# Quantus-Network/qp-zk-circuits

Measured on AMD Instinct MI355X. Metric: Wormhole proofs/sec, higher is better.
Workload: dtype u64

## Files before the change

include/qpgpu.h:

```cpp
#ifndef QPGPU_H
#define QPGPU_H
#include <stddef.h>
#include <stdint.h>

#ifdef __cplusplus
extern "C" {
#endif

typedef struct qpgpu_ctx qpgpu_ctx;
typedef struct qpgpu_circuit qpgpu_circuit;

enum {
    QPGPU_OK = 0,
    QPGPU_EINVAL = -1,
    QPGPU_EDEVICE = -2,
    QPGPU_ENOMEM = -3,
    QPGPU_EUNSAT = -4,
    QPGPU_EBUFSIZE = -5
};

int qpgpu_ctx_create(int device, qpgpu_ctx **out);
void qpgpu_ctx_destroy(qpgpu_ctx *ctx);
const char *qpgpu_last_error(const qpgpu_ctx *ctx);
int qpgpu_ctx_set_stream(qpgpu_ctx *ctx, void *hip_stream);
// ... 40 lines not shown
                           unsigned log_leaves, unsigned cap_height, uint64_t *d_digests, uint64_t *h_cap_out);
int qpgpu_merkle_build_rows_dev(qpgpu_ctx *ctx, const uint64_t *d_rows, uint32_t width, unsigned log_leaves,
                                unsigned cap_height, uint64_t *d_digests, uint64_t *h_cap_out);

int qpgpu_circuit_load(qpgpu_ctx *ctx, const uint64_t *pack_words, size_t n_words, qpgpu_circuit **out);
int qpgpu_circuit_load_batch(qpgpu_ctx *ctx, const uint64_t *pack_words, size_t n_words, unsigned max_batch, qpgpu_circuit **out);
unsigned qpgpu_circuit_max_batch(const qpgpu_circuit *c);
size_t qpgpu_circuit_num_public_inputs(const qpgpu_circuit *c);
void qpgpu_circuit_free(qpgpu_circuit *c);
int qpgpu_circuit_scrub(qpgpu_circuit *c);
int qpgpu_circuit_constants_sigmas_cap(const qpgpu_circuit *c, uint64_t *out, size_t out_words);
int qpgpu_circuit_set_blinding_seed(qpgpu_circuit *c, uint64_t seed);
int qpgpu_circuit_set_witness_check(qpgpu_circuit *c, int on);
int qpgpu_circuit_set_quotient_fused(qpgpu_circuit *c, int on);
int qpgpu_circuit_quotient_info(const qpgpu_circuit *c, int *fused_enabled, int *fused_selected);
size_t qpgpu_proof_size(const qpgpu_circuit *c);
int qpgpu_prove(qpgpu_circuit *c, const uint64_t *wires, const uint64_t *public_inputs, uint8_t *out, size_t out_cap, size_t *out_len);
int qpgpu_prove_dev(qpgpu_circuit *c, const uint64_t *d_wires, const uint64_t *public_inputs, uint8_t *out, size_t out_cap, size_t *out_len);
int qpgpu_prove_batch_dev(qpgpu_circuit *c, const uint64_t *const *d_wires, uint32_t batch, const uint64_t *const *public_inputs,
                          uint8_t *const *outs, size_t out_cap, size_t *out_lens);

int qpgpu_witness_info(qpgpu_circuit *c, uint64_t *num_generators, uint64_t *num_levels, uint64_t *num_free_cells);
int qpgpu_witness_free_mask(qpgpu_circuit *c, uint8_t *mask, size_t mask_len);
int qpgpu_generate_witness_dev(qpgpu_circuit *c, uint64_t *d_wires, const uint64_t *public_inputs);
int qpgpu_generate_witness(qpgpu_circuit *c, uint64_t *wires, const uint64_t *public_inputs);
int qpgpu_circuit_gate_rows(const qpgpu_circuit *c, unsigned gate_type, uint32_t *rows_out, size_t cap, size_t *count);
int qpgpu_generate_witness_batch_dev(qpgpu_circuit *c, uint64_t *d_wires, uint32_t batch, const uint64_t *public_inputs);
int qpgpu_generate_witness_partial_dev(qpgpu_circuit *c, const uint64_t *cells, const uint64_t *values, size_t count,
                                       const uint64_t *public_inputs, uint64_t *d_wires);
int qpgpu_generate_witness_partial_batch_dev(qpgpu_circuit *c, const uint64_t *cells, size_t count, const uint64_t *values,
// ... 143 lines not shown
```

integration/qpgpu_backend.rs:

```rust

use anyhow::{anyhow, bail, Result};
use core::ffi::{c_char, c_void};
use plonky2::field::extension::Extendable;
use plonky2::field::polynomial::PolynomialCoeffs;
use plonky2::field::types::PrimeField64;
use plonky2::hash::hash_types::RichField;
use plonky2::iop::target::Target;
use plonky2::iop::witness::{PartialWitness, PartitionWitness};
use plonky2::plonk::circuit_data::{CircuitData, CommonCircuitData, ProverOnlyCircuitData};
use plonky2::plonk::config::GenericConfig;
use plonky2::plonk::proof::ProofWithPublicInputs;

#[repr(C)] pub struct QpgpuCtx { _p: [u8; 0] }
#[repr(C)] pub struct QpgpuCircuit { _p: [u8; 0] }
#[repr(C)] pub struct QpgpuOracle { _p: [u8; 0] }
#[repr(C)] pub struct QpgpuStagePlan { _p: [u8; 0] }
#[repr(C)] pub struct QpgpuFriSession { _p: [u8; 0] }
#[repr(C)] pub struct QpgpuChallenger { pub sponge_state: [u64; 12], pub input_buffer: [u64; 8], pub output_buffer: [u64; 8], pub input_len: u32, pub output_len: u32 }
#[repr(C)] pub struct QpgpuFriRange { pub oracle: u32, pub first: u32, pub count: u32 }
#[repr(C)] pub struct QpgpuFriBatch { pub point: [u64; 2], pub num_ranges: u32, pub ranges: [QpgpuFriRange; 8] }
#[repr(C)] pub struct QpgpuFriParams { pub rate_bits: u32, pub cap_height: u32, pub proof_of_work_bits: u32, pub num_query_rounds: u32,
                                       pub num_reduction_rounds: u32, pub reduction_arity_bits: [u32; 16] }
pub const QPGPU_STAGE_ERR_CAP: usize = 256;

// ... 3 lines not shown
#[link(name = "qpgpu")]
extern "C" {
    pub fn qpgpu_ctx_create(device: i32, out: *mut *mut QpgpuCtx) -> i32;
    pub fn qpgpu_ctx_destroy(ctx: *mut QpgpuCtx);
    pub fn qpgpu_last_error(ctx: *const QpgpuCtx) -> *const c_char;
    pub fn qpgpu_ctx_pci_bus_id(ctx: *const QpgpuCtx, out: *mut c_char, out_len: usize) -> i32;
    pub fn qpgpu_ctx_set_hasher(ctx: *mut QpgpuCtx, kind: i32, params: *const u64, n_words: usize) -> i32;
    pub fn qpgpu_malloc(ctx: *mut QpgpuCtx, bytes: usize, dptr: *mut *mut c_void) -> i32;
    pub fn qpgpu_free(ctx: *mut QpgpuCtx, dptr: *mut c_void) -> i32;
    pub fn qpgpu_free_scrubbed(ctx: *mut QpgpuCtx, dptr: *mut c_void, bytes: usize) -> i32;
    pub fn qpgpu_memcpy_h2d(ctx: *mut QpgpuCtx, dst: *mut c_void, src: *const c_void, bytes: usize) -> i32;
    pub fn qpgpu_circuit_load_batch(ctx: *mut QpgpuCtx, pack: *const u64, n_words: usize, max_batch: u32, out: *mut *mut QpgpuCircuit) -> i32;
    pub fn qpgpu_circuit_free(c: *mut QpgpuCircuit);
    pub fn qpgpu_circuit_scrub(c: *mut QpgpuCircuit) -> i32;
    pub fn qpgpu_circuit_set_witness_check(c: *mut QpgpuCircuit, on: i32) -> i32;
    pub fn qpgpu_proof_size(c: *const QpgpuCircuit) -> usize;
    pub fn qpgpu_prove(c: *mut QpgpuCircuit, wires: *const u64, public_inputs: *const u64, out: *mut u8, out_cap: usize, out_len: *mut usize) -> i32;
    pub fn qpgpu_generate_witness_partial_dev(c: *mut QpgpuCircuit, cells: *const u64, values: *const u64, count: usize,
                                              public_inputs: *const u64, d_wires: *mut u64) -> i32;
    pub fn qpgpu_prove_dev(c: *mut QpgpuCircuit, d_wires: *const u64, public_inputs: *const u64, out: *mut u8, out_cap: usize, out_len: *mut usize) -> i32;
    pub fn qpgpu_prove_batch_dev(c: *mut QpgpuCircuit, d_wires: *const *const u64, batch: u32, public_inputs: *const *const u64,
                                 outs: *const *mut u8, out_cap: usize, out_lens: *mut usize) -> i32;
    pub fn qpgpu_pack_validate(pack: *const u64, n_words: usize, err: *mut c_char) -> i32;
    pub fn qpgpu_stage_plan_create(ctx: *mut QpgpuCtx, words: *const u64, n_words: usize, cs_oracle: *const QpgpuOracle,
                                   out: *mut *mut QpgpuStagePlan, err: *mut c_char) -> i32;
    pub fn qpgpu_stage_plan_free(plan: *mut QpgpuStagePlan);
    pub fn qpgpu_stage_plan_info(plan: *const QpgpuStagePlan, degree_bits: *mut u32, num_challenges: *mut u32, num_partial_products: *mut u32,
                                 quotient_degree_factor: *mut u32, fused_selected: *mut i32) -> i32;
    pub fn qpgpu_stage_partial_products(plan: *mut QpgpuStagePlan, wires: *const u64, wires_on_device: i32, betas: *const u64,
                                        gammas: *const u64, d_out: *mut u64) -> i32;
// ... 537 lines not shown
```

qp-zk-circuits_amd/binding.py:

```python
import ctypes
import os

import numpy as np

P = 0xFFFFFFFF00000001
MULT_GEN = 14293326489335486720

NTT_FORWARD = 0
NTT_INVERSE = 1
NTT_OUT_BITREV = 2

_HERE = os.path.dirname(os.path.abspath(__file__))


def lib_path():
    return os.path.join(_HERE, "libqpgpu.so")


class QpGpuError(RuntimeError):
    def __init__(self, code, msg):
        super().__init__(f"qpgpu error {code}: {msg}")
        self.code = code


# ... 68 lines not shown
        "qpgpu_circuit_max_batch": (c.c_uint, [vp]),
        "qpgpu_circuit_scrub": (c.c_int, [vp]),
        "qpgpu_prove_batch_dev": (c.c_int, [vp, vp, c.c_uint32, vp, vp, c.c_size_t, vp]),
        "qpgpu_ctx_set_hasher": (c.c_int, [vp, c.c_int, u64p, c.c_size_t]),
        "qpgpu_ctx_get_hasher": (c.c_int, [vp]),
        "qpgpu_ctx_challenger_observe": (c.c_int, [vp, vp, u64p, c.c_size_t]),
        "qpgpu_ctx_challenger_get": (c.c_int, [vp, vp, c.POINTER(c.c_uint64)]),
        "qpgpu_pool_create_batched": (c.c_int, [c.c_int, u64p, c.c_size_t, c.c_uint, c.c_uint, c.POINTER(vp)]),
        "qpgpu_circuit_free": (None, [vp]),
        "qpgpu_circuit_constants_sigmas_cap": (c.c_int, [vp, u64p, c.c_size_t]),
        "qpgpu_proof_size": (c.c_size_t, [vp]),
        "qpgpu_circuit_set_blinding_seed": (c.c_int, [vp, c.c_uint64]),
        "qpgpu_circuit_set_witness_check": (c.c_int, [vp, c.c_int]),
        "qpgpu_circuit_set_quotient_fused": (c.c_int, [vp, c.c_int]),
        "qpgpu_circuit_quotient_info": (c.c_int, [vp, c.POINTER(c.c_int), c.POINTER(c.c_int)]),
        "qpgpu_circuit_gate_rows": (c.c_int, [vp, c.c_uint, vp, c.c_size_t, c.POINTER(c.c_size_t)]),
        "qpgpu_prove": (c.c_int, [vp, u64p, u64p, vp, c.c_size_t, c.POINTER(c.c_size_t)]),
        "qpgpu_prove_dev": (c.c_int, [vp, u64p, u64p, vp, c.c_size_t, c.POINTER(c.c_size_t)]),
        "qpgpu_poseidon_constants": (c.c_size_t, [u64p, u64p, c.c_size_t]),
        "qpgpu_pool_create": (c.c_int, [c.c_int, u64p, c.c_size_t, c.c_uint, c.POINTER(vp)]),
        "qpgpu_pool_destroy": (None, [vp]),
        "qpgpu_pool_proof_size": (c.c_size_t, [vp]),
        "qpgpu_pool_workers": (c.c_uint, [vp]),
        "qpgpu_pool_last_error": (c.c_char_p, [vp]),
        "qpgpu_pool_submit": (c.c_int, [vp, u64p, u64p, vp, c.c_size_t, c.POINTER(c.c_uint64)]),
        "qpgpu_pool_wait": (c.c_int, [vp, c.c_uint64, c.POINTER(c.c_size_t)]),
        "qpgpu_pool_set_witness_check": (c.c_int, [vp, c.c_int]),
        "qpgpu_pool_create_multi": (c.c_int, [vp, c.c_uint, u64p, c.c_size_t, c.c_uint, c.c_uint, c.c_uint, c.POINTER(vp)]),
        "qpgpu_pool_devices": (c.c_uint, [vp]),
        "qpgpu_pool_serialized": (c.c_int, [vp]),
# ... 357 lines not shown

    def proof_size(self):
        return self.gpu.lib.qpgpu_proof_size(self.h)

    def set_witness_check(self, on=True):
        self.gpu._check(self.gpu.lib.qpgpu_circuit_set_witness_check(self.h, 1 if on else 0))

    def set_quotient_fused(self, on=True):
        self.gpu._check(self.gpu.lib.qpgpu_circuit_set_quotient_fused(self.h, 1 if on else 0))

    def quotient_info(self):
        a, b = ctypes.c_int(), ctypes.c_int()
        self.gpu._check(self.gpu.lib.qpgpu_circuit_quotient_info(self.h, ctypes.byref(a), ctypes.byref(b)))
        return bool(a.value), bool(b.value)

    def set_blinding_seed(self, seed):
        self.gpu._check(self.gpu.lib.qpgpu_circuit_set_blinding_seed(self.h, seed))

    def constants_sigmas_cap(self, cap_height=4):
        out = np.empty((1 << cap_height, 4), dtype=np.uint64)
        self.gpu._check(self.gpu.lib.qpgpu_circuit_constants_sigmas_cap(self.h, out.ctypes.data, out.size))
        return out

    def witness_info(self):
        a, b, c3 = ctypes.c_uint64(), ctypes.c_uint64(), ctypes.c_uint64()
        self.gpu._check(self.gpu.lib.qpgpu_witness_info(self.h, ctypes.byref(a), ctypes.byref(b), ctypes.byref(c3)))
        return a.value, b.value, c3.value

    def gate_rows(self, gate_type):
        n = ctypes.c_size_t()
# ... 761 lines not shown
```

qp-zk-circuits_amd/csrc/prover.cpp:

```cpp
#include <hip/hip_runtime.h>
#include <algorithm>
#include <array>
#include <cstring>
#include <random>
#include <string>
#include <vector>
#include "circuit.hpp"
#include "ctx.hpp"
#include "gl64.hpp"
#include "merkle.hpp"
#include "poseidon.hpp"
#include "prover_host.hpp"
#include "circuit_state.hpp"
#include "prover_kernels.hpp"

using gl::e2;
using gl::u64;

namespace {

int alloc_batch(qpgpu_circuit *c, PolyOracle &b, uint32_t ncols, uint32_t nb, bool need_coeffs = true, uint32_t oracle_index = 0) {
    const CircuitPack &p = c->pack;
    const u64 n = p.n(), lde_n = n << p.rate_bits;
    const bool secret = oracle_index > 0;
// ... 158 lines not shown
}

int qpgpu_circuit_set_quotient_fused(qpgpu_circuit *c, int on) {
    if (!c) return QPGPU_EINVAL;
    c->tab.quotient_fused = on != 0;
    return QPGPU_OK;
}

int qpgpu_circuit_quotient_info(const qpgpu_circuit *c, int *fused_enabled, int *fused_selected) {
    if (!c) return QPGPU_EINVAL;
    if (fused_enabled) *fused_enabled = c->tab.quotient_fused ? 1 : 0;
    if (fused_selected) *fused_selected = c->tab.fused_selected(c->pack) ? 1 : 0;
    return QPGPU_OK;
}

int qpgpu_circuit_set_blinding_seed(qpgpu_circuit *c, uint64_t seed) {
    if (!c) return QPGPU_EINVAL;
    c->blinding_seed = seed; c->seed_set = true;
    return QPGPU_OK;
}

int qpgpu_circuit_constants_sigmas_cap(const qpgpu_circuit *c, uint64_t *out, size_t out_words) {
    if (!c || !out || out_words < c->cs.cap.size()) return QPGPU_EINVAL;
    std::memcpy(out, c->cs.cap.data(), c->cs.cap.size() * 8);
    return QPGPU_OK;
}

}

static int prove_batch_impl(qpgpu_circuit *c, uint32_t nb, const u64 *d_wires, const u64 *const *public_inputs, uint8_t *const *outs, size_t out_cap, size_t *out_lens) {
// ... 184 lines not shown
```

qp-zk-circuits_amd/csrc/prover_stages.cpp:

```cpp
#include <hip/hip_runtime.h>
#include <cstdlib>
#include <cstring>
#include "gl64.hpp"
#include "poseidon.hpp"
#include "prover_stages.hpp"

using gl::u64;

namespace {

std::vector<u64> powers_table(u64 base, u64 count) {
    std::vector<u64> t(count);
    u64 a = 1;
    for (u64 i = 0; i < count; i++) { t[i] = gl::canon(a); a = gl::mul(a, base); }
    return t;
}

struct SmallLayout {
    size_t nch, R, nterms, betas, gammas, bk, apow, pih;
    explicit SmallLayout(const CircuitPack &p) {
        nch = p.num_challenges; R = p.num_routed_wires;
        nterms = nch + nch * p.num_chunks() + p.num_gate_constraints;
        betas = 0; gammas = nch; bk = 2 * nch; apow = bk + nch * R; pih = apow + nch * nterms;
    }
// ... 5 lines not shown
    const u64 n = p.n();
    const uint32_t nch = (uint32_t)p.num_challenges, nchunks = (uint32_t)p.num_chunks();
    PpArgs pa{};
    pa.wires = d_wires; pa.sigmas = t.cs_values + (p.num_selectors + p.num_constants) * n; pa.omega_pows = t.d_omega; pa.beta_k_is = w.d_small + sl.bk;
    pa.betas = w.d_small + sl.betas; pa.gammas = w.d_small + sl.gammas; pa.qcp = w.d_qcp; pa.rowprod = w.d_rowprod; pa.n = n;
    pa.num_routed = (uint32_t)p.num_routed_wires; pa.chunk = (uint32_t)p.quotient_degree_factor; pa.nchunks = nchunks; pa.nch = nch;
    pa.batch = nb; pa.ps_wires = ps_wires; pa.ps_small = t.small_words; pa.ps_qcp = (u64)nch * nchunks * n; pa.ps_rowprod = (u64)nch * n;
    return pa;
}

}

bool StageTables::fused_selected(const CircuitPack &p) const {
    return quotient_fused && pk_quotient_fused_gates(h_gates.data(), (uint32_t)h_gates.size(), (uint32_t)p.num_routed_wires,
                                                     (uint32_t)p.quotient_degree_factor, (uint32_t)p.num_partial_products + 1, nullptr);
}

std::string stage_limits(const CircuitPack &p) {
    if (p.num_chunks() > 16 || p.num_challenges > 4) return "too many chunks/challenges";
    if (p.degree_bits + p.rate_bits > 23) return "LDE larger than 2^23 not supported";
    if (p.degree_bits + p.rate_bits > 20 && p.rate_bits > 3) return "an LDE beyond 2^20 points needs rate_bits <= 3";
    return "";
}

int h2d_sync(qpgpu_ctx *ctx, void *dst, const void *src, size_t bytes) {
    QP_HIP(ctx, hipMemcpyAsync(dst, src, bytes, hipMemcpyHostToDevice, ctx->stream));
    QP_HIP(ctx, hipStreamSynchronize(ctx->stream));
    return QPGPU_OK;
}

// ... 35 lines not shown
        if (e != hipSuccess) return ctx->hip_fail(e, "coset_tables");
        const u64 ginv = gl::inv(gl::MULT_GEN);
        t.ginv_lo_bits = lo_bits;
        auto glo = powers_table(ginv, 1ull << lo_bits), ghi = powers_table(gl::pow(ginv, 1ull << lo_bits), 1ull << (L - lo_bits));
        QP_TRY(alloc(&t.d_ginv_lo, glo.size(), false)); QP_TRY(alloc(&t.d_ginv_hi, ghi.size(), false));
        QP_TRY(h2d_sync(ctx, t.d_ginv_lo, glo.data(), glo.size() * 8)); QP_TRY(h2d_sync(ctx, t.d_ginv_hi, ghi.data(), ghi.size() * 8));
    }
    t.small_words = SmallLayout(p).words();
    {
        const uint32_t n_hash = pk_count_hash_gates(gd.data(), (uint32_t)gd.size());
        const char *e = getenv("QPGPU_QUOTIENT_FOLD");
        if (n_hash > 0 && n_hash <= qfold::MAX_GATES && !(e && *e == '0')) t.fold_words = (size_t)n_hash * p.num_challenges * qfold::WORDS;
    }
    if (const char *e = getenv("QPGPU_QUOTIENT_FUSED")) if (*e == '0') t.quotient_fused = false;
    if (const char *e = getenv("QPGPU_QUOTIENT_XCD_MAP")) if (*e == '0') t.quotient_plain_map = true;
    return QPGPU_OK;
}

int stage_work_alloc(const CircuitPack &p, const StageTables &t, const StageAlloc &alloc, uint32_t B, StageWork &w) {
    const u64 n = p.n(), lde_n = n << p.rate_bits, nch = p.num_challenges;
    QP_TRY(alloc(&w.d_qacc, (size_t)B * nch * lde_n, true));
    QP_TRY(alloc(&w.d_qcp, (size_t)B * nch * p.num_chunks() * n, true));
    QP_TRY(alloc(&w.d_rowprod, (size_t)B * nch * n, true));
    QP_TRY(alloc(&w.d_z, (size_t)B * nch * n, true));
    QP_TRY(alloc(&w.d_small, (size_t)B * t.small_words, false));
    if (t.fold_words) QP_TRY(alloc(&w.d_fold, (size_t)B * t.fold_words, false));
    QP_TRY(alloc(&w.d_check, (size_t)B * 2, false));
    return QPGPU_OK;
}

// ... 55 lines not shown
    QP_TRY(w.stage->put_rows(ctx, d_apow, SW, small + sl.apow, SW, (size_t)nch * nterms + 4, nb));
    QuotientArgs qa{};
    qa.alpha_pows = d_apow; qa.poseidon_rc = t.d_poseidon_rc; qa.p2_gate = ctx->d_p2_app; qa.p2_layout = p.p2_layout;
    qa.nch = nch; qa.nchunks = nchunks; qa.nterms = (uint32_t)nterms; qa.num_gates = (uint32_t)p.gates.size(); qa.batch = nb; qa.ps_small = SW;
    qa.fold = w.d_fold; qa.ps_fold = t.fold_words;
    QP_HIP(ctx, pk_quotient_fold_sweep(qa, t.h_gates.data(), st));
    if (v.check_wires) {
        QuotientArgs ta{};
        ta.wires = v.check_wires; ta.cs = t.cs_values; ta.alpha_pows = d_apow; ta.pi_hash = d_pih; ta.gates = t.d_gates;
        ta.acc = w.d_qacc; ta.out = w.d_qacc; ta.poseidon_rc = t.d_poseidon_rc;
        ta.p2_gate = ctx->d_p2_app; ta.p2_layout = p.p2_layout;
        ta.zh_inv = t.d_zh_inv; ta.lde_n = n; ta.q_n = n; ta.q_shift = 0; ta.log_lde = d; ta.rate = 1; ta.nch = nch; ta.num_routed = (uint32_t)R;
        ta.chunk = (uint32_t)p.quotient_degree_factor; ta.nchunks = nchunks; ta.sig0 = (uint32_t)sig0;
        ta.num_selectors = (uint32_t)p.num_selectors; ta.num_gates = (uint32_t)p.gates.size(); ta.nterms = (uint32_t)nterms;
        ta.batch = nb; ta.ps_wires = v.ps_check_wires; ta.ps_zs = 0; ta.ps_small = SW; ta.ps_acc = (u64)nch * n; ta.ps_out = (u64)nch * n;
        ta.fold = w.d_fold; ta.ps_fold = t.fold_words;
        QP_HIP(ctx, hipMemsetAsync(w.d_qacc, 0, (size_t)nb * nch * n * 8, st));
        std::vector<u64> init(2 * (size_t)nb);
        for (uint32_t b = 0; b < nb; b++) { init[2 * b] = ~0ull; init[2 * b + 1] = 0; }
        QP_TRY(w.stage->put(ctx, w.d_check, init.data(), init.size() * 8));
        QP_HIP(ctx, pk_gate_sums(ta, t.h_gates.data(), st));
        QP_HIP(ctx, pk_witness_check(w.d_qacc, n, nch, w.d_z, w.d_rowprod, w.d_check, nb, st));
        std::vector<u64> res(2 * (size_t)nb);
        QP_TRY(ctx->read_back(res.data(), w.d_check, res.size() * 8));
        for (uint32_t b = 0; b < nb; b++) {
            const std::string who = nb > 1 ? " (proof " + std::to_string(b) + " of the batch)" : "";
            if (res[2 * b] != ~0ull) return ctx->fail(QPGPU_EUNSAT, "witness does not satisfy the circuit: gate constraints fail at row " + std::to_string(res[2 * b]) + who);
            if (res[2 * b + 1]) return ctx->fail(QPGPU_EUNSAT, "witness does not satisfy the circuit: a copy constraint is violated (permutation product != 1)" + who);
        }
    }
    ctx->prof_begin("prove_quotient");
    qa.wires = v.wires_lde; qa.cs = t.cs_lde; qa.zs_pp = v.zs_lde; qa.x_coset = t.d_x_coset; qa.l0_coset = t.d_l0_coset;
    qa.zh_inv = t.d_zh_inv; qa.alpha_pows = d_apow; qa.beta_k_is = d_bk; qa.betas = d_betas; qa.gammas = d_gammas; qa.pi_hash = d_pih;
    qa.gates = t.d_gates; qa.acc = w.d_qacc; qa.poseidon_rc = t.d_poseidon_rc; qa.out = v.out;
    qa.p2_gate = ctx->d_p2_app; qa.p2_layout = p.p2_layout; qa.lde_n = lde_n; qa.q_n = q_n; qa.q_shift = q_shift; qa.log_lde = L; qa.rate = 1u << p.rate_bits; qa.nch = nch;
    qa.num_routed = (uint32_t)R; qa.chunk = (uint32_t)p.quotient_degree_factor; qa.nchunks = nchunks; qa.sig0 = (uint32_t)sig0;
    qa.num_selectors = (uint32_t)p.num_selectors; qa.num_gates = (uint32_t)p.gates.size(); qa.nterms = (uint32_t)nterms;
    qa.batch = nb; qa.ps_wires = v.ps_wires_lde; qa.ps_zs = v.ps_zs_lde; qa.ps_small = SW; qa.ps_acc = (u64)nch * lde_n; qa.ps_out = (u64)nch * q_n;
    qa.fused = t.quotient_fused ? 1 : 0; qa.fused_plain_map = t.quotient_plain_map ? 1 : 0;
    QP_HIP(ctx, pk_quotient(qa, t.h_gates.data(), st));
    QP_TRY(ntt_run(ctx, v.out, v.out, Lq, Lq, (size_t)nch * nb, true, false, 0));
    QP_HIP(ctx, pk_scale_powers(v.out, q_n, (u64)nch * nb, t.d_ginv_lo, t.d_ginv_hi, t.ginv_lo_bits, st));
    ctx->prof_end();
    return QPGPU_OK;
}
```

qp-zk-circuits_amd/csrc/prover_stages.hpp:

```cpp
#pragma once
#include <hip/hip_runtime_api.h>
#include <functional>
#include <string>
#include <vector>
#include "circuit.hpp"
#include "ctx.hpp"
#include "prover_host.hpp"
#include "prover_kernels.hpp"

using StageAlloc = std::function<int(gl::u64 **p, size_t count, bool secret)>;

struct StageTables {
    const gl::u64 *cs_values = nullptr, *cs_lde = nullptr;
    GateDev *d_gates = nullptr;
    std::vector<GateDev> h_gates;
    bool has_p2_gate = false;
    gl::u64 *d_poseidon_rc = nullptr;
    gl::u64 *d_omega = nullptr, *d_x_coset = nullptr, *d_l0_coset = nullptr, *d_zh_inv = nullptr;
    gl::u64 *d_ginv_lo = nullptr, *d_ginv_hi = nullptr; uint32_t ginv_lo_bits = 0;
    size_t small_words = 0;
    size_t fold_words = 0;
    bool quotient_fused = true;
    bool quotient_plain_map = false;
    bool fused_selected(const CircuitPack &p) const;
};

struct StageWork {
    gl::u64 *d_small = nullptr, *d_fold = nullptr;
    gl::u64 *d_qcp = nullptr, *d_rowprod = nullptr, *d_z = nullptr;
    gl::u64 *d_qacc = nullptr;
    gl::u64 *d_check = nullptr;
    Stager *stage = nullptr;
};

std::string stage_limits(const CircuitPack &p);
int h2d_sync(qpgpu_ctx *ctx, void *dst, const void *src, size_t bytes);
int stage_tables_build(qpgpu_ctx *ctx, const CircuitPack &p, const StageAlloc &alloc, StageTables &t);
int stage_work_alloc(const CircuitPack &p, const StageTables &t, const StageAlloc &alloc, uint32_t max_batch, StageWork &w);
size_t stage_ring_words(const StageTables &t, uint32_t max_batch);
// ... 18 lines not shown
```

qp-zk-circuits_amd/csrc/quotient_fold.hpp:

```cpp
#pragma once
#include "circuit.hpp"
#include "gl64.hpp"
#include "poseidon.hpp"

#if defined(__HIP_DEVICE_COMPILE__)
#define QFOLD_UNROLL _Pragma("unroll")
#else
#define QFOLD_UNROLL
#endif

namespace qfold {
using gl::u32;
using gl::u64;

enum Lin : u32 { LIN_MDS = 0, LIN_P2_EXT = 1, LIN_P2_INT = 2 };
enum Head : u32 { HEAD_SBOX = 0, HEAD_RAW = 1 };

struct Schedule {
    u32 kind;
    u32 head;
    u32 q0;
    u32 nw;
    u32 nseg;
    u32 run_wire[3], run_len[3];
    u32 w_input, w_output, w_swap, w_delta;
};
constexpr u32 NO_SWAP = P2GateLayout::NO_SWAP;
constexpr u32 T_HEAD = 0, T_OMEGA = 12, T_NALPHA = 130, T_KAPPA = 260, WORDS = 264;
constexpr u32 MAX_GATES = 2;

inline Schedule poseidon_schedule() {
    Schedule s{};
    s.kind = GATE_POSEIDON; s.head = HEAD_SBOX; s.q0 = 5; s.nw = 106; s.nseg = 30;
    s.run_wire[0] = 29; s.run_len[0] = 36; s.run_wire[1] = 65; s.run_len[1] = 22; s.run_wire[2] = 87; s.run_len[2] = 48;
    s.w_input = 0; s.w_output = 12; s.w_swap = 24; s.w_delta = 25;
    return s;
}
inline Schedule poseidon2_schedule(const P2GateLayout &lay) {
    Schedule s{};
    s.kind = GATE_POSEIDON2; s.head = lay.first_round_wires ? HEAD_RAW : HEAD_SBOX; s.q0 = lay.has_swap() ? 5 : 0;
    s.run_wire[0] = lay.w_full0; s.run_len[0] = 12 * lay.full0_rounds(); s.run_wire[1] = lay.w_partial; s.run_len[1] = 22;
    s.run_wire[2] = lay.w_full1; s.run_len[2] = 48;
    s.nw = s.run_len[0] + 70; s.nseg = lay.first_round_wires ? 31 : 30;
    s.w_input = lay.w_input; s.w_output = lay.w_output; s.w_swap = lay.w_swap; s.w_delta = lay.w_delta;
    return s;
}

struct Consts { const u64 *rc; const poseidon2::Params *p2; };

GL_HD int seg_round(const Schedule &s, int k) { return k - (s.head == HEAD_RAW ? 1 : 0); }
GL_HD u32 seg_targets(const Schedule &s, int k) { const int r = seg_round(s, k); return r >= 3 && r <= 24 ? 1u : 12u; }
GL_HD u32 seg_lin(const Schedule &s, int k) {
    if (s.kind == GATE_POSEIDON) return LIN_MDS;
    const int r = seg_round(s, k);
    return r >= 4 && r <= 25 ? LIN_P2_INT : LIN_P2_EXT;
}
GL_HD u64 seg_rc(const Schedule &s, const Consts &c, int k, int i) {
    const int r = seg_round(s, k);
    if (r == 29) return 0;
    if (s.kind == GATE_POSEIDON) return c.rc[(u32)((r + 1) * 12 + i)];
// ... 116 lines not shown
}

GL_HD u64 folded_sum(const Schedule &s, const Consts &c, const u64 *row, const u64 *ap, const u64 *table) {
    u64 sum = table[T_KAPPA], st[12];
    swapped_inputs(s, [&](u32 w) { return row[w]; }, [&](u32 q, u64 cst) { sum = gl::add(sum, gl::mul(ap[q], cst)); }, st);
    head_inputs(s, c, st);
    for (int i = 0; i < 12; i++) sum = gl::add(sum, gl::mul(table[T_HEAD + i], s.head == HEAD_SBOX ? poseidon::sbox7(st[i]) : st[i]));
    for (u32 j = 0; j < s.nw; j++) {
        const u64 v = row[target_wire(s, j)];
        sum = gl::add(sum, gl::add(gl::mul(table[T_OMEGA + j], poseidon::sbox7(v)), gl::mul(table[T_NALPHA + j], v)));
    }
    for (int i = 0; i < 12; i++) sum = gl::add(sum, gl::mul(table[T_NALPHA + s.nw + i], row[s.w_output + i]));
    return gl::canon(sum);
}

#undef QFOLD_UNROLL
}
```

qp-zk-circuits_amd/csrc/quotient_kernels.hip:

```cpp
#include <hip/hip_runtime.h>
#include "gl64.hpp"
#include "poseidon.hpp"
#include "quotient_kernels.hpp"
#include "quotient_map.hpp"

using gl::e2;
using gl::u32;
using gl::u64;

namespace {

__device__ __forceinline__ u64 gate_filter(const QuotientArgs &a, u32 gi, u64 s) {
    const GateDev g = a.gates[gi];
    u64 f = 1;
    for (u32 j = g.group_start; j < g.group_end; j++)
        if (j != gi) f = gl::mul(f, gl::sub((u64)j, s));
    if (a.num_selectors > 1) f = gl::mul(f, gl::sub(0xFFFFFFFFull, s));
    return f;
}


__device__ __forceinline__ void quotient_select_proof(QuotientArgs &a) {
    const u64 pr = blockIdx.z;
    a.wires += pr * a.ps_wires; a.zs_pp += pr * a.ps_zs;
// ... 520 lines not shown
    u64 sum[NCH];
#pragma unroll
    for (int c = 0; c < NCH; c++) sum[c] = gl::add(gl::acc_reduce(wsum[c]), F[c * qfold::WORDS + qfold::T_KAPPA]);
    quotient_add_store(a, S, j, f, sum, finalize);
}
template <int NCH>
__global__ void __launch_bounds__(256) quotient_poseidon_kernel(QuotientArgs a, qfold::Schedule s, u32 gi, u32 t0, u32 slot, int finalize) {
    s.kind = GATE_POSEIDON; s.head = qfold::HEAD_SBOX;
    hash_gate_folded<NCH>(a, s, gi, t0, slot, finalize);
}
template <int NCH>
__global__ void __launch_bounds__(256) quotient_poseidon2_kernel(QuotientArgs a, qfold::Schedule s, u32 gi, u32 t0, u32 slot, int finalize) {
    s.kind = GATE_POSEIDON2;
    hash_gate_folded<NCH>(a, s, gi, t0, slot, finalize);
}
__global__ void __launch_bounds__(64) quotient_fold_sweep_kernel(FoldSweepArgs fa) {
    __shared__ qfold::Scratch scratch;
    const u32 slot = blockIdx.x, c = blockIdx.y;
    const u64 pr = blockIdx.z;
    const u64 *ap = fa.alpha_pows + pr * fa.ps_small + (u64)c * fa.nterms + fa.t0;
    u64 *table = fa.fold + pr * fa.ps_fold + ((u64)slot * fa.nch + c) * qfold::WORDS;
    const qfold::Consts K = {fa.poseidon_rc, fa.p2_gate};
    qfold::sweep(fa.sched[slot], K, ap, scratch, table, threadIdx.x, blockDim.x, [] { __syncthreads(); });
}

__global__ void __launch_bounds__(256) witness_check_kernel(const u64 *acc, u64 n, u32 nch, const u64 *z, const u64 *rowprod, u64 *result) {
    const u64 i = blockIdx.x * (u64)blockDim.x + threadIdx.x;
    if (i >= n) return;
    { const u64 pr = blockIdx.z; acc += pr * nch * n; z += pr * nch * n; rowprod += pr * nch * n; result += pr * 2; }
    bool bad = false;
// ... 18 lines not shown
}
static qfold::Schedule hash_gate_schedule(const QuotientArgs &a, const GateDev &g) {
    return g.type == GATE_POSEIDON ? qfold::poseidon_schedule() : qfold::poseidon2_schedule(a.p2_layout);
}
template <int NCH>
static void hash_gate_launch(const QuotientArgs &a, const GateDev *host_gates, u32 gi, u32 t0, u32 slot, int finalize, dim3 g, dim3 b, hipStream_t st) {
    const bool p1 = host_gates[gi].type == GATE_POSEIDON;
    const qfold::Schedule s = hash_gate_schedule(a, host_gates[gi]);
    if (a.fold) {
        if (p1) hipLaunchKernelGGL((quotient_poseidon_kernel<NCH>), g, b, 0, st, a, s, gi, t0, slot, finalize);
        else hipLaunchKernelGGL((quotient_poseidon2_kernel<NCH>), g, b, 0, st, a, s, gi, t0, slot, finalize);
    } else {
        if (p1) hipLaunchKernelGGL((quotient_hash_rounds_kernel<NCH, GATE_POSEIDON>), g, b, 0, st, a, s, gi, t0, finalize);
        else hipLaunchKernelGGL((quotient_hash_rounds_kernel<NCH, GATE_POSEIDON2>), g, b, 0, st, a, s, gi, t0, finalize);
    }
}
hipError_t pk_quotient_fold_sweep(const QuotientArgs &a, const GateDev *host_gates, hipStream_t st) {
    if (!a.fold || a.batch == 0) return hipSuccess;
    FoldSweepArgs fa{};
    for (u32 i = 0; i < a.num_gates; i++)
        if (is_hash_gate(host_gates[i])) {
            if (fa.ngates == qfold::MAX_GATES) return hipErrorInvalidValue;
            fa.sched[fa.ngates++] = hash_gate_schedule(a, host_gates[i]);
        }
    if (fa.ngates == 0) return hipSuccess;
    fa.nch = a.nch; fa.nterms = a.nterms; fa.t0 = a.nch + a.nch * a.nchunks; fa.batch = a.batch;
    fa.alpha_pows = a.alpha_pows; fa.poseidon_rc = a.poseidon_rc; fa.p2_gate = a.p2_gate;
    fa.fold = const_cast<u64 *>(a.fold); fa.ps_small = a.ps_small; fa.ps_fold = a.ps_fold;
    hipLaunchKernelGGL(quotient_fold_sweep_kernel, dim3(fa.ngates, fa.nch, fa.batch), dim3(64), 0, st, fa);
    return hipGetLastError();
// ... 18 lines not shown
    dim3 b(256), g((unsigned)((a.q_n + 255) / 256), 1, a.batch);
    const u32 t0 = a.nch + a.nch * a.nchunks;
    const u32 n_hash = pk_count_hash_gates(host_gates, a.num_gates);
    const int fin_gates = finalize && n_hash == 0;
    FusedGates fg;
    const u32 tiles = g.x;
    const bool grouped = a.fused_plain_map == 0;
    if (perm && a.fused && pk_quotient_fused_gates(host_gates, a.num_gates, a.num_routed, a.chunk, a.nchunks, &fg) &&
        qmap::grid_size(tiles, a.batch, grouped) <= 0x7FFFFFFFull) {
        hipLaunchKernelGGL((quotient_perm_gates_kernel<NCH>), dim3((unsigned)qmap::grid_size(tiles, a.batch, grouped)), b, 0, st, a, fg, tiles, grouped ? 1u : 0u, fin_gates);
    } else {
        if (perm) hipLaunchKernelGGL((quotient_perm_kernel<NCH>), g, b, 0, st, a);
        if (wide_random_access(a, host_gates)) hipLaunchKernelGGL((quotient_gates_kernel<NCH, true>), g, b, 0, st, a, t0, fin_gates);
        else hipLaunchKernelGGL((quotient_gates_kernel<NCH, false>), g, b, 0, st, a, t0, fin_gates);
    }
    u32 slot = 0;
    for (u32 i = 0; i < a.num_gates; i++)
        if (is_hash_gate(host_gates[i])) {
            hash_gate_launch<NCH>(a, host_gates, i, t0, slot, finalize && slot + 1 == n_hash, g, b, st);
            slot++;
        }
    return hipGetLastError();
}
static hipError_t quotient_dispatch(const QuotientArgs &a, const GateDev *host_gates, bool perm, bool finalize, hipStream_t st) {
    switch (a.nch) {
        case 1: return quotient_launch<1>(a, host_gates, perm, finalize, st);
        case 2: return quotient_launch<2>(a, host_gates, perm, finalize, st);
        case 3: return quotient_launch<3>(a, host_gates, perm, finalize, st);
        case 4: return quotient_launch<4>(a, host_gates, perm, finalize, st);
        default: return hipErrorInvalidValue;
// ... 12 lines not shown
```

qp-zk-circuits_amd/csrc/quotient_kernels.hpp:

```cpp
#pragma once
#include <hip/hip_runtime.h>
#include <stdint.h>
#include "circuit.hpp"
#include "gl64.hpp"
#include "quotient_fold.hpp"

struct GateDev { uint32_t type, param0, param1, selector_index, group_start, group_end, num_constraints, param2; };

struct QuotientArgs {
    const uint64_t *wires, *cs, *zs_pp;
    const uint64_t *x_coset, *l0_coset;
    const uint64_t *zh_inv;
    const uint64_t *alpha_pows;
    const uint64_t *beta_k_is, *betas, *gammas, *pi_hash;
    const GateDev *gates;
    const uint64_t *poseidon_rc;
    const poseidon2::Params *p2_gate;
    P2GateLayout p2_layout;
    uint64_t *acc;
    uint64_t *out;
    uint64_t lde_n;
    uint64_t q_n;
    uint32_t q_shift;
    uint32_t log_lde, rate, nch, num_routed, chunk, nchunks, sig0, num_selectors, num_gates, nterms;
    uint32_t batch;
    uint64_t ps_wires, ps_zs, ps_small, ps_acc, ps_out;
    const uint64_t *fold;
    uint64_t ps_fold;
    uint32_t fused, fused_plain_map;
};

struct FusedGates { uint32_t constant, public_input, arithmetic, base_sum, n_consts, n_ops, n_limbs; };

struct FoldSweepArgs {
    qfold::Schedule sched[qfold::MAX_GATES];
    uint32_t ngates, nch, nterms, t0, batch;
    const uint64_t *alpha_pows;
    const uint64_t *poseidon_rc;
    const poseidon2::Params *p2_gate;
    uint64_t *fold;
    uint64_t ps_small, ps_fold;
};

hipError_t pk_quotient(const QuotientArgs &a, const GateDev *host_gates, hipStream_t st);
bool pk_quotient_fused_gates(const GateDev *host_gates, uint32_t num_gates, uint32_t num_routed, uint32_t chunk, uint32_t nchunks, FusedGates *out);
uint32_t pk_count_hash_gates(const GateDev *host_gates, uint32_t num_gates);
hipError_t pk_quotient_fold_sweep(const QuotientArgs &a, const GateDev *host_gates, hipStream_t st);
hipError_t pk_gate_sums(const QuotientArgs &a, const GateDev *host_gates, hipStream_t st);
hipError_t pk_witness_check(const uint64_t *acc, uint64_t n, uint32_t nch, const uint64_t *z, const uint64_t *rowprod, uint64_t *result, uint32_t batch, hipStream_t st);

__device__ __forceinline__ uint32_t brev32(uint32_t x, uint32_t bits) { return bits ? __brev(x) >> (32 - bits) : 0; }
```

Baseline: 1535.

## Evaluate paired Poseidon and Poseidon2 hash gates in one quotient kernel

When a circuit has exactly two hash gates, one Poseidon and one Poseidon2, with matching folded schedules, a single kernel now evaluates both. It reads the 106 target wires once, computes their sbox7 values once, and shares the linear accumulation, with a separate head per gate. This removes one full pass over the LDE wire columns and one kernel launch in the quotient stage. The cost is more accumulator registers per thread, which may lower occupancy. The path is on by default and can be turned off with QPGPU_QUOTIENT_PAIR=0.

```diff
diff --git a/include/qpgpu.h b/include/qpgpu.h
--- a/include/qpgpu.h
+++ b/include/qpgpu.h
@@ -78,6 +78,7 @@
 int qpgpu_circuit_set_witness_check(qpgpu_circuit *c, int on);
 int qpgpu_circuit_set_quotient_fused(qpgpu_circuit *c, int on);
 int qpgpu_circuit_quotient_info(const qpgpu_circuit *c, int *fused_enabled, int *fused_selected);
+int qpgpu_circuit_quotient_pair_info(const qpgpu_circuit *c, int *enabled, int *selected);
 size_t qpgpu_proof_size(const qpgpu_circuit *c);
 int qpgpu_prove(qpgpu_circuit *c, const uint64_t *wires, const uint64_t *public_inputs, uint8_t *out, size_t out_cap, size_t *out_len);
 int qpgpu_prove_dev(qpgpu_circuit *c, const uint64_t *d_wires, const uint64_t *public_inputs, uint8_t *out, size_t out_cap, size_t *out_len);
diff --git a/integration/qpgpu_backend.rs b/integration/qpgpu_backend.rs
--- a/integration/qpgpu_backend.rs
+++ b/integration/qpgpu_backend.rs
@@ -41,6 +41,7 @@
     pub fn qpgpu_circuit_free(c: *mut QpgpuCircuit);
     pub fn qpgpu_circuit_scrub(c: *mut QpgpuCircuit) -> i32;
     pub fn qpgpu_circuit_set_witness_check(c: *mut QpgpuCircuit, on: i32) -> i32;
+    pub fn qpgpu_circuit_quotient_pair_info(c: *const QpgpuCircuit, enabled: *mut i32, selected: *mut i32) -> i32;
     pub fn qpgpu_proof_size(c: *const QpgpuCircuit) -> usize;
     pub fn qpgpu_prove(c: *mut QpgpuCircuit, wires: *const u64, public_inputs: *const u64, out: *mut u8, out_cap: usize, out_len: *mut usize) -> i32;
     pub fn qpgpu_generate_witness_partial_dev(c: *mut QpgpuCircuit, cells: *const u64, values: *const u64, count: usize,
diff --git a/qp-zk-circuits_amd/binding.py b/qp-zk-circuits_amd/binding.py
--- a/qp-zk-circuits_amd/binding.py
+++ b/qp-zk-circuits_amd/binding.py
@@ -106,6 +106,7 @@
         "qpgpu_circuit_set_witness_check": (c.c_int, [vp, c.c_int]),
         "qpgpu_circuit_set_quotient_fused": (c.c_int, [vp, c.c_int]),
         "qpgpu_circuit_quotient_info": (c.c_int, [vp, c.POINTER(c.c_int), c.POINTER(c.c_int)]),
+        "qpgpu_circuit_quotient_pair_info": (c.c_int, [vp, c.POINTER(c.c_int), c.POINTER(c.c_int)]),
         "qpgpu_circuit_gate_rows": (c.c_int, [vp, c.c_uint, vp, c.c_size_t, c.POINTER(c.c_size_t)]),
         "qpgpu_prove": (c.c_int, [vp, u64p, u64p, vp, c.c_size_t, c.POINTER(c.c_size_t)]),
         "qpgpu_prove_dev": (c.c_int, [vp, u64p, u64p, vp, c.c_size_t, c.POINTER(c.c_size_t)]),
@@ -493,6 +494,11 @@
         self.gpu._check(self.gpu.lib.qpgpu_circuit_quotient_info(self.h, ctypes.byref(a), ctypes.byref(b)))
         return bool(a.value), bool(b.value)
 
+    def quotient_pair_info(self):
+        a, b = ctypes.c_int(), ctypes.c_int()
+        self.gpu._check(self.gpu.lib.qpgpu_circuit_quotient_pair_info(self.h, ctypes.byref(a), ctypes.byref(b)))
+        return bool(a.value), bool(b.value)
+
     def set_blinding_seed(self, seed):
         self.gpu._check(self.gpu.lib.qpgpu_circuit_set_blinding_seed(self.h, seed))
 
diff --git a/qp-zk-circuits_amd/csrc/prover.cpp b/qp-zk-circuits_amd/csrc/prover.cpp
--- a/qp-zk-circuits_amd/csrc/prover.cpp
+++ b/qp-zk-circuits_amd/csrc/prover.cpp
@@ -196,6 +196,13 @@
     return QPGPU_OK;
 }
 
+int qpgpu_circuit_quotient_pair_info(const qpgpu_circuit *c, int *enabled, int *selected) {
+    if (!c || !enabled || !selected) return QPGPU_EINVAL;
+    *enabled = c->tab.quotient_pair ? 1 : 0;
+    *selected = c->tab.pair_selected(c->pack) ? 1 : 0;
+    return QPGPU_OK;
+}
+
 int qpgpu_circuit_set_blinding_seed(qpgpu_circuit *c, uint64_t seed) {
     if (!c) return QPGPU_EINVAL;
     c->blinding_seed = seed; c->seed_set = true;
diff --git a/qp-zk-circuits_amd/csrc/prover_stages.cpp b/qp-zk-circuits_amd/csrc/prover_stages.cpp
--- a/qp-zk-circuits_amd/csrc/prover_stages.cpp
+++ b/qp-zk-circuits_amd/csrc/prover_stages.cpp
@@ -43,6 +43,10 @@
 bool StageTables::fused_selected(const CircuitPack &p) const {
     return quotient_fused && pk_quotient_fused_gates(h_gates.data(), (uint32_t)h_gates.size(), (uint32_t)p.num_routed_wires,
                                                      (uint32_t)p.quotient_degree_factor, (uint32_t)p.num_partial_products + 1, nullptr);
+}
+
+bool StageTables::pair_selected(const CircuitPack &p) const {
+    return quotient_pair && fold_words != 0 && pk_quotient_pairable(h_gates.data(), (uint32_t)h_gates.size(), p.p2_layout);
 }
 
 std::string stage_limits(const CircuitPack &p) {
@@ -108,6 +112,7 @@
     }
     if (const char *e = getenv("QPGPU_QUOTIENT_FUSED")) if (*e == '0') t.quotient_fused = false;
     if (const char *e = getenv("QPGPU_QUOTIENT_XCD_MAP")) if (*e == '0') t.quotient_plain_map = true;
+    if (const char *e = getenv("QPGPU_QUOTIENT_PAIR")) if (*e == '0') t.quotient_pair = false;
     return QPGPU_OK;
 }
 
@@ -193,7 +198,7 @@
         ta.chunk = (uint32_t)p.quotient_degree_factor; ta.nchunks = nchunks; ta.sig0 = (uint32_t)sig0;
         ta.num_selectors = (uint32_t)p.num_selectors; ta.num_gates = (uint32_t)p.gates.size(); ta.nterms = (uint32_t)nterms;
         ta.batch = nb; ta.ps_wires = v.ps_check_wires; ta.ps_zs = 0; ta.ps_small = SW; ta.ps_acc = (u64)nch * n; ta.ps_out = (u64)nch * n;
-        ta.fold = w.d_fold; ta.ps_fold = t.fold_words;
+        ta.fold = w.d_fold; ta.ps_fold = t.fold_words; ta.pair = t.quotient_pair ? 1 : 0;
         QP_HIP(ctx, hipMemsetAsync(w.d_qacc, 0, (size_t)nb * nch * n * 8, st));
         std::vector<u64> init(2 * (size_t)nb);
         for (uint32_t b = 0; b < nb; b++) { init[2 * b] = ~0ull; init[2 * b + 1] = 0; }
@@ -216,7 +221,7 @@
     qa.num_routed = (uint32_t)R; qa.chunk = (uint32_t)p.quotient_degree_factor; qa.nchunks = nchunks; qa.sig0 = (uint32_t)sig0;
     qa.num_selectors = (uint32_t)p.num_selectors; qa.num_gates = (uint32_t)p.gates.size(); qa.nterms = (uint32_t)nterms;
     qa.batch = nb; qa.ps_wires = v.ps_wires_lde; qa.ps_zs = v.ps_zs_lde; qa.ps_small = SW; qa.ps_acc = (u64)nch * lde_n; qa.ps_out = (u64)nch * q_n;
-    qa.fused = t.quotient_fused ? 1 : 0; qa.fused_plain_map = t.quotient_plain_map ? 1 : 0;
+    qa.fused = t.quotient_fused ? 1 : 0; qa.fused_plain_map = t.quotient_plain_map ? 1 : 0; qa.pair = t.quotient_pair ? 1 : 0;
     QP_HIP(ctx, pk_quotient(qa, t.h_gates.data(), st));
     QP_TRY(ntt_run(ctx, v.out, v.out, Lq, Lq, (size_t)nch * nb, true, false, 0));
     QP_HIP(ctx, pk_scale_powers(v.out, q_n, (u64)nch * nb, t.d_ginv_lo, t.d_ginv_hi, t.ginv_lo_bits, st));
diff --git a/qp-zk-circuits_amd/csrc/prover_stages.hpp b/qp-zk-circuits_amd/csrc/prover_stages.hpp
--- a/qp-zk-circuits_amd/csrc/prover_stages.hpp
+++ b/qp-zk-circuits_amd/csrc/prover_stages.hpp
@@ -22,7 +22,9 @@
     size_t fold_words = 0;
     bool quotient_fused = true;
     bool quotient_plain_map = false;
+    bool quotient_pair = true;
     bool fused_selected(const CircuitPack &p) const;
+    bool pair_selected(const CircuitPack &p) const;
 };
 
 struct StageWork {
diff --git a/qp-zk-circuits_amd/csrc/quotient_fold.hpp b/qp-zk-circuits_amd/csrc/quotient_fold.hpp
--- a/qp-zk-circuits_amd/csrc/quotient_fold.hpp
+++ b/qp-zk-circuits_amd/csrc/quotient_fold.hpp
@@ -29,7 +29,7 @@
 constexpr u32 T_HEAD = 0, T_OMEGA = 12, T_NALPHA = 130, T_KAPPA = 260, WORDS = 264;
 constexpr u32 MAX_GATES = 2;
 
-inline Schedule poseidon_schedule() {
+GL_HD Schedule poseidon_schedule() {
     Schedule s{};
     s.kind = GATE_POSEIDON; s.head = HEAD_SBOX; s.q0 = 5; s.nw = 106; s.nseg = 30;
     s.run_wire[0] = 29; s.run_len[0] = 36; s.run_wire[1] = 65; s.run_len[1] = 22; s.run_wire[2] = 87; s.run_len[2] = 48;
@@ -44,6 +44,13 @@
     s.nw = s.run_len[0] + 70; s.nseg = lay.first_round_wires ? 31 : 30;
     s.w_input = lay.w_input; s.w_output = lay.w_output; s.w_swap = lay.w_swap; s.w_delta = lay.w_delta;
     return s;
+}
+
+GL_HD bool pairable(const Schedule &a, const Schedule &b) {
+    if (!((a.kind == GATE_POSEIDON && b.kind == GATE_POSEIDON2) || (a.kind == GATE_POSEIDON2 && b.kind == GATE_POSEIDON))) return false;
+    if (a.head != HEAD_SBOX || b.head != HEAD_SBOX || a.q0 != b.q0 || a.nw != b.nw) return false;
+    for (int r = 0; r < 3; r++) if (a.run_wire[r] != b.run_wire[r] || a.run_len[r] != b.run_len[r]) return false;
+    return a.w_input == b.w_input && a.w_output == b.w_output && a.w_swap == b.w_swap && a.w_delta == b.w_delta;
 }
 
 struct Consts { const u64 *rc; const poseidon2::Params *p2; };
@@ -190,5 +197,24 @@
     return gl::canon(sum);
 }
 
+GL_HD u64 pair_sum(const Schedule &a, const Schedule &b, const Consts &c, const u64 *row, const u64 *ap, const u64 *ta, const u64 *tb, u64 fa, u64 fb) {
+    u64 lin = 0, oma = 0, omb = 0, st[12], h[12];
+    swapped_inputs(a, [&](u32 w) { return row[w]; }, [&](u32 q, u64 cst) { lin = gl::add(lin, gl::mul(ap[q], cst)); }, st);
+    for (int i = 0; i < 12; i++) h[i] = st[i];
+    head_inputs(a, c, h);
+    for (int i = 0; i < 12; i++) oma = gl::add(oma, gl::mul(ta[T_HEAD + i], poseidon::sbox7(h[i])));
+    head_inputs(b, c, st);
+    for (int i = 0; i < 12; i++) omb = gl::add(omb, gl::mul(tb[T_HEAD + i], poseidon::sbox7(st[i])));
+    for (u32 j = 0; j < a.nw; j++) {
+        const u64 v = row[target_wire(a, j)], y = poseidon::sbox7(v);
+        lin = gl::add(lin, gl::mul(ta[T_NALPHA + j], v));
+        oma = gl::add(oma, gl::mul(ta[T_OMEGA + j], y));
+        omb = gl::add(omb, gl::mul(tb[T_OMEGA + j], y));
+    }
+    for (int i = 0; i < 12; i++) lin = gl::add(lin, gl::mul(ta[T_NALPHA + a.nw + i], row[a.w_output + i]));
+    const u64 sa = gl::add(gl::add(oma, lin), ta[T_KAPPA]), sb = gl::add(gl::add(omb, lin), tb[T_KAPPA]);
+    return gl::canon(gl::add(gl::mul(fa, sa), gl::mul(fb, sb)));
+}
+
 #undef QFOLD_UNROLL
 }
diff --git a/qp-zk-circuits_amd/csrc/quotient_kernels.hip b/qp-zk-circuits_amd/csrc/quotient_kernels.hip
--- a/qp-zk-circuits_amd/csrc/quotient_kernels.hip
+++ b/qp-zk-circuits_amd/csrc/quotient_kernels.hip
@@ -558,6 +558,99 @@
     s.kind = GATE_POSEIDON2;
     hash_gate_folded<NCH>(a, s, gi, t0, slot, finalize);
 }
+#ifndef PAIR_GROUP
+#define PAIR_GROUP FOLD_GROUP
+#endif
+constexpr int PAIR_TAIL = 106 % PAIR_GROUP;
+static_assert(12 % PAIR_GROUP == 0 && PAIR_TAIL > 0, "whole groups in the head, one tail group behind the 106 target wires");
+__device__ __forceinline__ gl::Acc192 acc_sum(const gl::Acc192 &x, const gl::Acc192 &y) {
+    gl::Acc192 r;
+    r.lo = x.lo + y.lo;
+    const u64 c0 = r.lo < x.lo ? 1 : 0, h = x.hi + y.hi;
+    r.hi = h + c0;
+    r.top = x.top + y.top + (u32)(h < x.hi ? 1 : 0) + (u32)(r.hi < c0 ? 1 : 0);
+    return r;
+}
+template <int NCH>
+__device__ __forceinline__ void pair_head(const u64 (&st)[12], const u64 *F, gl::Acc192 (&om)[NCH]) {
+#pragma unroll
+    for (int g0 = 0; g0 < 12; g0 += PAIR_GROUP) {
+        u64 h[PAIR_GROUP];
+#pragma unroll
+        for (int i = 0; i < PAIR_GROUP; i++) h[i] = st[g0 + i];
+        sbox7_group(h);
+#pragma unroll
+        for (int i = 0; i < PAIR_GROUP; i++)
+#pragma unroll
+            for (int c = 0; c < NCH; c++) gl::acc_mul(om[c], h[i], F[c * qfold::WORDS + qfold::T_HEAD + g0 + i]);
+    }
+}
+template <int NCH, int N>
+__device__ __forceinline__ void pair_targets(const QuotientArgs &a, const qfold::Schedule &s, const u64 *FA, const u64 *FB, u64 j, u32 j0,
+                                             gl::Acc192 (&lin)[NCH], gl::Acc192 (&omA)[NCH], gl::Acc192 (&omB)[NCH]) {
+    u64 v[N];
+#pragma unroll
+    for (int i = 0; i < N; i++) v[i] = a.wires[(u64)qfold::target_wire(s, j0 + i) * a.lde_n + j];
+#pragma unroll
+    for (int i = 0; i < N; i++)
+#pragma unroll
+        for (int c = 0; c < NCH; c++) gl::acc_mul(lin[c], v[i], a.fold[c * qfold::WORDS + qfold::T_NALPHA + j0 + i]);
+    sbox7_group(v);
+#pragma unroll
+    for (int i = 0; i < N; i++)
+#pragma unroll
+        for (int c = 0; c < NCH; c++) {
+            gl::acc_mul(omA[c], v[i], FA[c * qfold::WORDS + qfold::T_OMEGA + j0 + i]);
+            gl::acc_mul(omB[c], v[i], FB[c * qfold::WORDS + qfold::T_OMEGA + j0 + i]);
+        }
+}
+template <int NCH>
+__global__ void __launch_bounds__(256, NCH <= 2 ? 4 : 2) quotient_hash_pair_kernel(QuotientArgs a, u32 giA, u32 giB, u32 slotA, u32 slotB, u32 t0, int finalize) {
+    const u64 j = blockIdx.x * (u64)blockDim.x + threadIdx.x;
+    if (j >= a.q_n) return;
+    quotient_select_proof(a);
+    const u64 S = a.lde_n;
+    const u64 *ap = a.alpha_pows + t0;
+    const u64 *FA = a.fold + (u64)slotA * NCH * qfold::WORDS, *FB = a.fold + (u64)slotB * NCH * qfold::WORDS;
+    const qfold::Consts K = {a.poseidon_rc, a.p2_gate};
+    const qfold::Schedule s = qfold::poseidon_schedule();
+    qfold::Schedule sB = s;
+    sB.kind = GATE_POSEIDON2;
+    gl::Acc192 lin[NCH], omA[NCH], omB[NCH];
+#pragma unroll
+    for (int c = 0; c < NCH; c++) { lin[c] = gl::acc_zero(); omA[c] = gl::acc_zero(); omB[c] = gl::acc_zero(); }
+    u64 st[12];
+    qfold::swapped_inputs(s, WireAt{a.wires, S, j}, WeighInto<NCH>{lin, ap, a.nterms}, st);
+    {
+        u64 h[12];
+#pragma unroll
+        for (int i = 0; i < 12; i++) h[i] = st[i];
+        qfold::head_inputs(s, K, h);
+        pair_head<NCH>(h, FA, omA);
+    }
+    qfold::head_inputs(sB, K, st);
+    pair_head<NCH>(st, FB, omB);
+    u32 j0 = 0;
+#pragma unroll 1
+    for (; j0 + PAIR_GROUP <= s.nw; j0 += PAIR_GROUP) pair_targets<NCH, PAIR_GROUP>(a, s, FA, FB, j, j0, lin, omA, omB);
+    pair_targets<NCH, PAIR_TAIL>(a, s, FA, FB, j, j0, lin, omA, omB);
+#pragma unroll
+    for (int i = 0; i < 12; i++) {
+        const u64 o = a.wires[(u64)(s.w_output + i) * S + j];
+#pragma unroll
+        for (int c = 0; c < NCH; c++) gl::acc_mul(lin[c], o, a.fold[c * qfold::WORDS + qfold::T_NALPHA + s.nw + i]);
+    }
+    const u64 fA = gate_filter(a, giA, a.cs[(u64)a.gates[giA].selector_index * S + j]);
+    const u64 fB = gate_filter(a, giB, a.cs[(u64)a.gates[giB].selector_index * S + j]);
+    u64 sum[NCH];
+#pragma unroll
+    for (int c = 0; c < NCH; c++) {
+        const u64 gA = gl::add(gl::acc_reduce(acc_sum(omA[c], lin[c])), FA[c * qfold::WORDS + qfold::T_KAPPA]);
+        const u64 gB = gl::add(gl::acc_reduce(acc_sum(omB[c], lin[c])), FB[c * qfold::WORDS + qfold::T_KAPPA]);
+        sum[c] = gl::add(gl::mul(fA, gA), gl::mul(fB, gB));
+    }
+    quotient_add_store(a, S, j, 1, sum, finalize);
+}
 __global__ void __launch_bounds__(64) quotient_fold_sweep_kernel(FoldSweepArgs fa) {
     __shared__ qfold::Scratch scratch;
     const u32 slot = blockIdx.x, c = blockIdx.y;
@@ -606,6 +699,18 @@
         if (p1) hipLaunchKernelGGL((quotient_hash_rounds_kernel<NCH, GATE_POSEIDON>), g, b, 0, st, a, s, gi, t0, finalize);
         else hipLaunchKernelGGL((quotient_hash_rounds_kernel<NCH, GATE_POSEIDON2>), g, b, 0, st, a, s, gi, t0, finalize);
     }
+}
+static bool hash_gate_pair(const GateDev *host_gates, u32 num_gates, const P2GateLayout &lay, u32 (&idx)[2]) {
+    u32 n = 0;
+    for (u32 i = 0; i < num_gates; i++)
+        if (is_hash_gate(host_gates[i])) { if (n == 2) return false; idx[n++] = i; }
+    if (n != 2) return false;
+    auto sched = [&](u32 i) { return host_gates[i].type == GATE_POSEIDON ? qfold::poseidon_schedule() : qfold::poseidon2_schedule(lay); };
+    return qfold::pairable(sched(idx[0]), sched(idx[1]));
+}
+bool pk_quotient_pairable(const GateDev *host_gates, uint32_t num_gates, const P2GateLayout &p2_layout) {
+    u32 idx[2];
+    return hash_gate_pair(host_gates, num_gates, p2_layout, idx);
 }
 hipError_t pk_quotient_fold_sweep(const QuotientArgs &a, const GateDev *host_gates, hipStream_t st) {
     if (!a.fold || a.batch == 0) return hipSuccess;
@@ -654,6 +759,12 @@
         if (wide_random_access(a, host_gates)) hipLaunchKernelGGL((quotient_gates_kernel<NCH, true>), g, b, 0, st, a, t0, fin_gates);
         else hipLaunchKernelGGL((quotient_gates_kernel<NCH, false>), g, b, 0, st, a, t0, fin_gates);
     }
+    u32 pr[2];
+    if (a.fold && a.pair && hash_gate_pair(host_gates, a.num_gates, a.p2_layout, pr)) {
+        const u32 sa = host_gates[pr[0]].type == GATE_POSEIDON ? 0 : 1;
+        hipLaunchKernelGGL((quotient_hash_pair_kernel<NCH>), g, b, 0, st, a, pr[sa], pr[sa ^ 1], sa, sa ^ 1, t0, finalize ? 1 : 0);
+        return hipGetLastError();
+    }
     u32 slot = 0;
     for (u32 i = 0; i < a.num_gates; i++)
         if (is_hash_gate(host_gates[i])) {
diff --git a/qp-zk-circuits_amd/csrc/quotient_kernels.hpp b/qp-zk-circuits_amd/csrc/quotient_kernels.hpp
--- a/qp-zk-circuits_amd/csrc/quotient_kernels.hpp
+++ b/qp-zk-circuits_amd/csrc/quotient_kernels.hpp
@@ -28,6 +28,7 @@
     const uint64_t *fold;
     uint64_t ps_fold;
     uint32_t fused, fused_plain_map;
+    uint32_t pair;
 };
 
 struct FusedGates { uint32_t constant, public_input, arithmetic, base_sum, n_consts, n_ops, n_limbs; };
@@ -45,6 +46,7 @@
 hipError_t pk_quotient(const QuotientArgs &a, const GateDev *host_gates, hipStream_t st);
 bool pk_quotient_fused_gates(const GateDev *host_gates, uint32_t num_gates, uint32_t num_routed, uint32_t chunk, uint32_t nchunks, FusedGates *out);
 uint32_t pk_count_hash_gates(const GateDev *host_gates, uint32_t num_gates);
+bool pk_quotient_pairable(const GateDev *host_gates, uint32_t num_gates, const P2GateLayout &p2_layout);
 hipError_t pk_quotient_fold_sweep(const QuotientArgs &a, const GateDev *host_gates, hipStream_t st);
 hipError_t pk_gate_sums(const QuotientArgs &a, const GateDev *host_gates, hipStream_t st);
 hipError_t pk_witness_check(const uint64_t *acc, uint64_t n, uint32_t nch, const uint64_t *z, const uint64_t *rowprod, uint64_t *result, uint32_t batch, hipStream_t st);
```

Result: faster. 1591 (median of 6 runs) (+3.7%).
